# amirkdv/biseqt

Hardware: AMD Instinct MI355X
Metric: GCUPS (DP cell updates/s) banded local align (higher is better)
Workload: dtype i16

## Files before the change

biseqt_amd/_pwlib.py:

```python
import ctypes as C
import os

HERE = os.path.dirname(os.path.abspath(__file__))
PWLIB_SO = os.environ.get('PWLIB_SO', os.path.join(HERE, 'pwlib', 'pwlib.so'))
PWLIB_H = os.path.join(HERE, 'pwlib', 'pwlib.h')

STD_MODE, BANDED_MODE = 0, 1
GLOBAL, LOCAL, START_ANCHORED, END_ANCHORED, OVERLAP, START_ANCHORED_OVERLAP, \
    END_ANCHORED_OVERLAP = range(7)
B_GLOBAL, B_LOCAL, B_OVERLAP = range(3)


class intpair(C.Structure):
    _fields_ = [('i', C.c_int), ('j', C.c_int)]


class alnscores(C.Structure):
    _fields_ = [('subst_scores', C.POINTER(C.POINTER(C.c_double))),
                ('gap_open_score', C.c_double),
                ('gap_extend_score', C.c_double)]


class alnframe(C.Structure):
    _fields_ = [('origin', C.POINTER(C.c_int)),
# ... 37 lines not shown
class dptable(C.Structure):
    _fields_ = [('cells', C.POINTER(C.POINTER(dpcell))),
                ('num_rows', C.c_int),
                ('row_lens', C.POINTER(C.c_int)),
                ('prob', C.POINTER(alnprob))]


class alignment(C.Structure):
    _fields_ = [('origin_idx', C.c_int),
                ('mutant_idx', C.c_int),
                ('score', C.c_double),
                ('transcript', C.c_char_p)]


class pw_scoring(C.Structure):
    _fields_ = [('mode', C.c_int), ('type', C.c_int), ('alphabet_len', C.c_int),
                ('subst', C.POINTER(C.c_double)), ('go', C.c_double), ('ge', C.c_double)]


class pw_pair(C.Structure):
    _fields_ = [('origin_off', C.c_uint64), ('mutant_off', C.c_uint64),
                ('origin_len', C.c_int32), ('mutant_len', C.c_int32),
                ('dmin', C.c_int32), ('dmax', C.c_int32)]


class pw_result(C.Structure):
    _fields_ = [('score', C.c_double), ('opt_i', C.c_int32), ('opt_j', C.c_int32),
                ('origin_idx', C.c_int32), ('mutant_idx', C.c_int32),
                ('tx_len', C.c_int32), ('status', C.c_int32)]


PW_ST_TRACED, PW_ST_EMPTY, PW_ST_PANICK, PW_ST_BADPATH = 1, 2, 4, 8
PW_FLAG_DUMP_SCORES, PW_FLAG_FORCE_F64, PW_FLAG_FORCE_GENERIC, PW_FLAG_PROFILE = 1, 2, 4, 8
PW_FLAG_NO_PACKED16 = 16
PW_FLAG_FORCE_TILED = 32
PW_FLAG_FORCE_STRIP = 64
PW_FLAG_SHARED_ARENA = 128
PW_FLAG_NO_STRIP = 256

SIZEOF = dict(intpair=8, alnscores=24, alnframe=32, std_alnparams=4, banded_alnparams=12,
              alnprob=32, alnchoice=32, dpcell=16, dptable=32, alignment=24,
              pw_scoring=40, pw_pair=32, pw_result=32)

EXPORTS = ['dptable_init', 'dptable_solve', 'dptable_traceback', 'dptable_free',
           'pw_last_error', 'pw_device_count', 'pw_device_memory', 'pw_pool_trim', 'pw_batch_create', 'pw_batch_destroy',
           'pw_batch_init_rc', 'pw_batch_band', 'pw_batch_pair_cells', 'pw_batch_cells',
           'pw_batch_algorithmic_bytes', 'pw_batch_score_type', 'pw_batch_kernel_name', 'pw_batch_upload_arena',
           'pw_batch_arena_device', 'pw_arena_upload', 'pw_arena_free', 'pw_batch_share_arena', 'pw_host_alloc', 'pw_host_free', 'pw_batch_upload_arena_async',
           'pw_batch_results_async', 'pw_batch_transcripts_async', 'pw_batch_solve', 'pw_batch_traceback',
           'pw_batch_traceback_from', 'pw_batch_sync', 'pw_batch_results_device',
           'pw_batch_transcripts_device', 'pw_batch_transcripts_bytes', 'pw_batch_tx_slot',
           'pw_batch_results', 'pw_batch_transcripts', 'pw_batch_scores', 'pw_batch_masks', 'pw_batch_table', 'pw_batch_fill_ms',
           'pw_batch_trace_ms', 'pw_batch_pack_transcripts', 'pw_batch_packed_device', 'pw_batch_packed_offsets_device',
           'pw_batch_packed_total_async', 'pw_batch_packed', 'pw_plan_only']
SEED_EXPORTS = ['pw_seeds_create', 'pw_seeds_build', 'pw_seeds_num_rows', 'pw_seeds_is_self', 'pw_seeds_rows_device',
                'pw_seeds_rows', 'pw_seeds_count', 'pw_seeds_kmers', 'pw_seeds_band_neighbours', 'pw_seeds_graph_build', 'pw_seeds_graph_num_points', 'pw_seeds_graph_points',
                'pw_seeds_graph_counts', 'pw_seeds_graph_fetch', 'pw_seeds_graph_components', 'pw_seeds_build_ms',
                'pw_seeds_algorithmic_bytes', 'pw_seeds_destroy', 'pw_seeds_last_error']

MSEED_EXPORTS = ['pw_mseeds_create', 'pw_mseeds_build', 'pw_mseeds_num_seqs', 'pw_mseeds_num_rows', 'pw_mseeds_rows_device',
                 'pw_mseeds_rows', 'pw_mseeds_count_many', 'pw_mseeds_graph_build', 'pw_mseeds_graph_counts',
                 'pw_mseeds_graph_fetch', 'pw_mseeds_graph_components', 'pw_mseeds_build_ms', 'pw_mseeds_graph_ms',
                 'pw_mseeds_components_ms', 'pw_mseeds_count_ms', 'pw_mseeds_algorithmic_bytes', 'pw_mseeds_destroy',
                 'pw_mseeds_last_error']

OVERLAP_EXPORTS = ['pw_overlap_bands', 'pw_overlap_all_pairs', 'pw_overlap_last_ms', 'pw_overlap_last_error']


class pw_read_pair(C.Structure):
    _fields_ = [('s_off', C.c_uint64), ('t_off', C.c_uint64), ('s_len', C.c_int32), ('t_len', C.c_int32)]


def check_layout():
    for name, size in SIZEOF.items():
        assert C.sizeof(globals()[name]) == size, (name, C.sizeof(globals()[name]), size)


_lib = None


def _bind_hip_runtime():
    import sys
    choice = os.environ.get('PWLIB_HIP_RUNTIME', '')
    if choice == 'system':
        return None
    try:
        with open('/proc/self/maps') as f:
            if 'libamdhip64' in f.read():
                return None
    except OSError:
        pass
    path = choice
    if not path:
        if 'torch' in sys.modules:
            return None
        try:
            import importlib.util
            spec = importlib.util.find_spec('torch')
        except (ImportError, ValueError):
            spec = None
        if spec is None or not spec.origin:
            return None
        path = os.path.join(os.path.dirname(spec.origin), 'lib', 'libamdhip64.so')
    if not os.path.exists(path):
        return None
    try:
        return C.CDLL(path, mode=C.RTLD_GLOBAL)
# ... 31 lines not shown
    lib.pw_batch_band.argtypes = [C.c_void_p, C.c_int32, P(C.c_int32), P(C.c_int32), P(C.c_int32)]
    lib.pw_batch_pair_cells.argtypes = [C.c_void_p, C.c_int32]
    lib.pw_batch_pair_cells.restype = C.c_int64
    lib.pw_batch_cells.argtypes = [C.c_void_p]
    lib.pw_batch_cells.restype = C.c_int64
    lib.pw_batch_algorithmic_bytes.argtypes = [C.c_void_p]
    lib.pw_batch_algorithmic_bytes.restype = C.c_int64
    lib.pw_batch_score_type.argtypes = [C.c_void_p]
    lib.pw_batch_kernel_name.argtypes = [C.c_void_p]
    lib.pw_batch_kernel_name.restype = C.c_char_p
    lib.pw_batch_upload_arena.argtypes = [C.c_void_p, C.c_void_p, C.c_uint64]
    lib.pw_batch_arena_device.argtypes = [C.c_void_p]
    lib.pw_batch_arena_device.restype = C.c_void_p
    lib.pw_arena_upload.argtypes = [C.c_int, C.c_void_p, C.c_uint64]
    lib.pw_arena_upload.restype = C.c_void_p
    lib.pw_arena_free.argtypes = [C.c_int, C.c_void_p]
    lib.pw_arena_free.restype = None
    lib.pw_batch_share_arena.argtypes = [C.c_void_p, C.c_void_p]
    lib.pw_host_alloc.argtypes = [C.c_uint64]
    lib.pw_host_alloc.restype = C.c_void_p
    lib.pw_host_free.argtypes = [C.c_void_p]
    lib.pw_host_free.restype = None
    lib.pw_batch_upload_arena_async.argtypes = [C.c_void_p, C.c_void_p, C.c_uint64, C.c_void_p]
    lib.pw_batch_results_async.argtypes = [C.c_void_p, C.c_void_p, C.c_void_p]
    lib.pw_batch_transcripts_async.argtypes = [C.c_void_p, C.c_void_p, C.c_void_p]
    lib.pw_batch_solve.argtypes = [C.c_void_p, C.c_void_p]
    lib.pw_batch_traceback.argtypes = [C.c_void_p, C.c_void_p]
    lib.pw_batch_traceback_from.argtypes = [C.c_void_p, P(C.c_int32), C.c_void_p]
    lib.pw_batch_sync.argtypes = [C.c_void_p, C.c_void_p]
    lib.pw_batch_results_device.argtypes = [C.c_void_p]
    lib.pw_batch_results_device.restype = C.c_void_p
    lib.pw_batch_transcripts_device.argtypes = [C.c_void_p]
    lib.pw_batch_transcripts_device.restype = C.c_void_p
    lib.pw_batch_transcripts_bytes.argtypes = [C.c_void_p]
    lib.pw_batch_transcripts_bytes.restype = C.c_uint64
    lib.pw_batch_tx_slot.argtypes = [C.c_void_p, C.c_int32, P(C.c_uint64), P(C.c_int32)]
    lib.pw_batch_results.argtypes = [C.c_void_p, C.c_void_p]
    lib.pw_batch_transcripts.argtypes = [C.c_void_p, C.c_void_p]
    lib.pw_batch_scores.argtypes = [C.c_void_p, C.c_int32, P(C.c_double), C.c_int64]
    lib.pw_batch_table.argtypes = [C.c_void_p, C.c_int32, P(C.c_double), C.c_int64]
    lib.pw_batch_masks.argtypes = [C.c_void_p, C.c_int32, P(C.c_uint8), C.c_int64]
    lib.pw_batch_fill_ms.argtypes = [C.c_void_p]
    lib.pw_batch_fill_ms.restype = C.c_float
    lib.pw_batch_trace_ms.argtypes = [C.c_void_p]
    lib.pw_batch_trace_ms.restype = C.c_float
    lib.pw_batch_pack_transcripts.argtypes = [C.c_void_p, C.c_void_p]
    lib.pw_batch_packed_device.argtypes = [C.c_void_p]
    lib.pw_batch_packed_device.restype = C.c_void_p
    lib.pw_batch_packed_offsets_device.argtypes = [C.c_void_p]
    lib.pw_batch_packed_offsets_device.restype = C.c_void_p
    lib.pw_batch_packed_total_async.argtypes = [C.c_void_p, C.c_void_p, C.c_void_p]
    lib.pw_batch_packed.argtypes = [C.c_void_p, C.c_void_p, C.c_uint64, C.c_void_p]
    lib.pw_plan_only.argtypes = [P(pw_scoring), C.c_int32, P(pw_pair), C.c_uint64, C.c_uint32, C.c_char_p, C.c_int32, P(C.c_int32)]
    lib.pw_seeds_create.argtypes = [C.c_int, C.c_void_p, C.c_int64, C.c_void_p, C.c_int64, C.c_int, C.c_int,
                                    P(C.c_uint64), C.c_int, C.c_int]
    lib.pw_seeds_create.restype = C.c_void_p
    lib.pw_seeds_build.argtypes = [C.c_void_p, C.c_int64, C.c_void_p]
    lib.pw_seeds_num_rows.argtypes = [C.c_void_p]
    lib.pw_seeds_num_rows.restype = C.c_int64
    lib.pw_seeds_is_self.argtypes = [C.c_void_p]
    lib.pw_seeds_rows_device.argtypes = [C.c_void_p]
    lib.pw_seeds_rows_device.restype = C.c_void_p
    lib.pw_seeds_rows.argtypes = [C.c_void_p, C.c_void_p, C.c_int64]
    lib.pw_seeds_count.argtypes = [C.c_void_p, C.c_int, C.c_int32, C.c_int32, C.c_int, C.c_int32, C.c_int32]
    lib.pw_seeds_count.restype = C.c_int64
    lib.pw_seeds_kmers.argtypes = [C.c_void_p, C.c_int, C.c_void_p, C.c_int64]
    lib.pw_seeds_kmers.restype = C.c_int64
    lib.pw_seeds_band_neighbours.argtypes = [C.c_void_p, C.c_void_p, C.c_int64, C.c_void_p, C.c_int64]
    lib.pw_seeds_graph_build.argtypes = [C.c_void_p, C.c_double, C.c_double]
    lib.pw_seeds_graph_build.restype = C.c_int64
    lib.pw_seeds_graph_num_points.argtypes = [C.c_void_p]
    lib.pw_seeds_graph_num_points.restype = C.c_int64
    lib.pw_seeds_graph_points.argtypes = [C.c_void_p, C.c_void_p, C.c_int64]
    lib.pw_seeds_graph_counts.argtypes = [C.c_void_p, C.c_void_p, C.c_int64]
    lib.pw_seeds_graph_fetch.argtypes = [C.c_void_p, C.c_void_p, C.c_void_p]
    lib.pw_seeds_graph_components.argtypes = [C.c_void_p, C.c_void_p, C.c_void_p]
    lib.pw_seeds_build_ms.argtypes = [C.c_void_p]
    lib.pw_seeds_build_ms.restype = C.c_double
    lib.pw_seeds_algorithmic_bytes.argtypes = [C.c_void_p]
    lib.pw_seeds_algorithmic_bytes.restype = C.c_int64
    lib.pw_seeds_destroy.argtypes = [C.c_void_p]
    lib.pw_seeds_destroy.restype = None
    lib.pw_seeds_last_error.restype = C.c_char_p
    lib.pw_mseeds_create.argtypes = [C.c_int, C.c_void_p, C.c_void_p, C.c_int, C.c_int, C.c_int]
    lib.pw_mseeds_create.restype = C.c_void_p
    lib.pw_mseeds_build.argtypes = [C.c_void_p, C.c_int64, C.c_void_p]
    lib.pw_mseeds_num_seqs.argtypes = [C.c_void_p]
    lib.pw_mseeds_num_rows.argtypes = [C.c_void_p]
    lib.pw_mseeds_num_rows.restype = C.c_int64
    lib.pw_mseeds_rows_device.argtypes = [C.c_void_p]
    lib.pw_mseeds_rows_device.restype = C.c_void_p
    lib.pw_mseeds_rows.argtypes = [C.c_void_p, C.c_void_p, C.c_int64]
    lib.pw_mseeds_count_many.argtypes = [C.c_void_p, C.c_int64, C.c_void_p, C.c_void_p, C.c_void_p, C.c_void_p]
    lib.pw_mseeds_graph_build.argtypes = [C.c_void_p, C.c_double, C.c_double]
    lib.pw_mseeds_graph_build.restype = C.c_int64
    lib.pw_mseeds_graph_counts.argtypes = [C.c_void_p, C.c_void_p, C.c_int64]
    lib.pw_mseeds_graph_fetch.argtypes = [C.c_void_p, C.c_void_p, C.c_void_p]
    lib.pw_mseeds_graph_components.argtypes = [C.c_void_p, C.c_void_p, C.c_void_p]
    for f in ('pw_mseeds_build_ms', 'pw_mseeds_graph_ms', 'pw_mseeds_components_ms', 'pw_mseeds_count_ms'):
        getattr(lib, f).argtypes = [C.c_void_p]
        getattr(lib, f).restype = C.c_double
    lib.pw_mseeds_algorithmic_bytes.argtypes = [C.c_void_p]
    lib.pw_mseeds_algorithmic_bytes.restype = C.c_int64
    lib.pw_mseeds_destroy.argtypes = [C.c_void_p]
    lib.pw_mseeds_destroy.restype = None
    lib.pw_mseeds_last_error.restype = C.c_char_p
# ... 14 lines not shown
```

biseqt_amd/csrc/pw_launch.h:

```cpp
#ifndef PW_LAUNCH_H
#define PW_LAUNCH_H

#include <hip/hip_runtime_api.h>

#include "pw_plan.h"
#include "pw_types.h"

namespace pw {

hipError_t launch_fill(const FillParams<int32_t>& a, int variant, int bk, int nblocks, hipStream_t st);
hipError_t launch_fill(const FillParams<double>& a, int variant, int bk, int nblocks, hipStream_t st);
hipError_t launch_fill16(const FillParams<int32_t>& a, int bk, int seg, int rule, int mat, int nwaves, hipStream_t st);
hipError_t launch_fill16_mw(const FillParams<int32_t>& a, int bk, int rule, int mat, int nw, int npairs, hipStream_t st);
hipError_t launch_fill_mw(const FillParams<int32_t>& a, int variant, int bk, int nw, int nblocks, hipStream_t st);
hipError_t launch_fill_mw(const FillParams<double>& a, int variant, int bk, int nw, int nblocks, hipStream_t st);
hipError_t launch_tile(const FillParams<int32_t>& a, int variant, int pair, int ntiles, hipStream_t st);
hipError_t launch_tile(const FillParams<double>& a, int variant, int pair, int ntiles, hipStream_t st);
hipError_t launch_tile_finish(const FillParams<int32_t>& a, int pair, hipStream_t st);
hipError_t launch_tile_finish(const FillParams<double>& a, int pair, hipStream_t st);
hipError_t launch_trace(const TraceParams& p, hipStream_t st);
hipError_t launch_tx_pack(const PairDesc* pairs, const Result* results, const uint8_t* slots, int n, uint64_t* offsets,
                          uint8_t* packed, hipStream_t st);
struct StripParams;
struct StripTraceParams;
hipError_t launch_strip_fill(const StripParams& a, bool track, bool byte_rows, const uint32_t* ctl_init, int nworkers, int lds_bytes,
                             hipStream_t st);
hipError_t launch_strip_trace(const StripTraceParams& p, hipStream_t st);
hipError_t launch_xcc_census(uint32_t* d_seen8, hipStream_t st);
hipError_t launch_table_rowmajor(const void* plane, bool f64, int X, int Y, int pitch, double mul, double* out, hipStream_t st);

}
#endif
```

biseqt_amd/csrc/pw_trace.hip:

```cpp
#include "pw_device.h"

#include <stdlib.h>

namespace pw {

__global__ __launch_bounds__(64) void k_trace(const TraceParams p, const int walkers) {
  __shared__ uint32_t win[64][WIN_WORDS + 1];
  const int pair = (int)blockIdx.x * walkers + (int)threadIdx.x;
  if ((int)threadIdx.x < walkers && pair < p.npairs) trace_walk(p, pair, win[threadIdx.x]);
}

__device__ inline uint32_t bytes_equal(uint32_t w, uint32_t c4) {
  const uint32_t v = w ^ c4;
  const uint32_t t = (v & 0x7f7f7f7fu) + 0x7f7f7f7fu;
  return ~(t | v | 0x7f7f7f7fu);
}
__global__ __launch_bounds__(64) void k_trace_fixup(const TraceParams p) {
  const int pair = (int)blockIdx.x;
  const PairDesc& pd = p.pairs[pair];
  if (!pd.solvable) return;
  const Result r = p.results[pair];
  if (!(r.status & ST_TRACED) || r.tx_len <= 0) return;
  const uint8_t* oseq = p.arena + pd.o_off;
  const uint8_t* mseq = p.arena + pd.m_off;
// ... 38 lines not shown
__global__ __launch_bounds__(1024) void k_tx_offsets(const Result* __restrict__ results, int n, unsigned long long* __restrict__ offsets) {
  __shared__ unsigned long long part[1024];
  const int t = (int)threadIdx.x;
  const int per = (n + 1023) / 1024;
  const int k0 = t * per, k1 = k0 + per < n ? k0 + per : n;
  unsigned long long s = 0;
  for (int k = k0; k < k1; k++) { const int len = results[k].tx_len; s += len > 0 ? (unsigned long long)len : 0ull; }
  part[t] = s;
  __syncthreads();
  for (int off = 1; off < 1024; off <<= 1) {
    const unsigned long long v = t >= off ? part[t - off] : 0ull;
    __syncthreads();
    part[t] += v;
    __syncthreads();
  }
  unsigned long long run = t > 0 ? part[t - 1] : 0ull;
  for (int k = k0; k < k1; k++) {
    offsets[k] = run;
    const int len = results[k].tx_len;
    run += len > 0 ? (unsigned long long)len : 0ull;
  }
  if (t == 1023) offsets[n] = part[1023];
}
__global__ __launch_bounds__(64) void k_tx_pack(const PairDesc* __restrict__ pairs, const Result* __restrict__ results,
                                                const uint8_t* __restrict__ slots, const unsigned long long* __restrict__ offsets,
                                                uint8_t* __restrict__ packed) {
  const int pair = (int)blockIdx.x;
  const int len = results[pair].tx_len;
  if (len <= 0) return;
  const PairDesc& pd = pairs[pair];
  const uint8_t* src = slots + pd.tx_off + pd.tx_cap - len;
  uint8_t* dst = packed + offsets[pair];
  const int lane = (int)threadIdx.x;
  const int head = (int)((4u - (uint32_t)((uintptr_t)dst & 3u)) & 3u);
  if (lane < head && lane < len) dst[lane] = src[lane];
  const int nwords = len > head ? (len - head) >> 2 : 0;
  for (int q = lane; q < nwords; q += 64) {
    const uint8_t* sp = src + head + 4 * q;
    PackedU32 v = *(const PackedU32*)sp;
    *(uint32_t*)(dst + head + 4 * q) = v.v;
  }
  const int tail0 = head + 4 * nwords;
  if (tail0 + lane < len) dst[tail0 + lane] = src[tail0 + lane];
}
hipError_t launch_tx_pack(const PairDesc* pairs, const Result* results, const uint8_t* slots, int n, uint64_t* offsets,
                          uint8_t* packed, hipStream_t st) {
  hipLaunchKernelGGL(k_tx_offsets, dim3(1), dim3(1024), 0, st, results, n, (unsigned long long*)offsets);
  hipError_t e = hipGetLastError();
  if (e != hipSuccess || n <= 0) return e;
  hipLaunchKernelGGL(k_tx_pack, dim3((unsigned)n), dim3(64), 0, st, pairs, results, slots, (const unsigned long long*)offsets, packed);
  return hipGetLastError();
}

template <typename T>
__global__ __launch_bounds__(256) void k_table_rowmajor(const T* __restrict__ plane, int X, int Y, int pitch, double mul, double* __restrict__ out) {
  const int64_t c = (int64_t)blockIdx.x * 256 + threadIdx.x;
  if (c >= (int64_t)(X + 1) * (Y + 1)) return;
  const int x = (int)(c / (Y + 1)), y = (int)(c - (int64_t)x * (Y + 1));
  out[c] = (double)plane[(int64_t)(x - y + Y) * pitch + (x < y ? x : y)] * mul;
}
hipError_t launch_table_rowmajor(const void* plane, bool f64, int X, int Y, int pitch, double mul, double* out, hipStream_t st) {
  const int64_t n = (int64_t)(X + 1) * (Y + 1);
  const dim3 grid((unsigned)((n + 255) / 256)), blk(256);
  if (f64) hipLaunchKernelGGL((k_table_rowmajor<double>), grid, blk, 0, st, (const double*)plane, X, Y, pitch, mul, out);
  else hipLaunchKernelGGL((k_table_rowmajor<int32_t>), grid, blk, 0, st, (const int32_t*)plane, X, Y, pitch, mul, out);
  return hipGetLastError();
}

hipError_t launch_trace(const TraceParams& p, hipStream_t st) {
  if (p.npairs <= 0) return hipSuccess;
  static int walkers = 0;
  if (walkers == 0) {
    const char* e = getenv("PWLIB_WALKERS_PER_WAVE");
    walkers = e ? atoi(e) : 64;
    if (walkers < 1 || walkers > 64) walkers = 64;
  }
  hipLaunchKernelGGL(k_trace, dim3((unsigned)((p.npairs + walkers - 1) / walkers)), dim3(64), 0, st, p, walkers);
  hipError_t e = hipGetLastError();
  if (e != hipSuccess) return e;
  hipLaunchKernelGGL(k_trace_fixup, dim3((unsigned)p.npairs, (unsigned)(p.fix_segments > 0 ? p.fix_segments : 1)), dim3(64), 0, st, p);
  return hipGetLastError();
}

#define PW_DECL(TN, T) \
  hipError_t launch_fill_##TN##_bk2(const FillParams<T>&, int, int, hipStream_t);  \
  hipError_t launch_fill_##TN##_bk4(const FillParams<T>&, int, int, hipStream_t);  \
  hipError_t launch_fill_##TN##_bk8(const FillParams<T>&, int, int, hipStream_t);  \
  hipError_t launch_fill_##TN##_bk16(const FillParams<T>&, int, int, hipStream_t); \
  hipError_t launch_fill_##TN##_bk32(const FillParams<T>&, int, int, hipStream_t);
PW_DECL(i32, int32_t)
PW_DECL(f64, double)
#undef PW_DECL
#define PW_BKS(M, R, MT) M(4, R, MT) M(8, R, MT) M(12, R, MT) M(16, R, MT) M(20, R, MT) M(24, R, MT) M(28, R, MT) M(32, R, MT)
#define PW_ALL16(M) PW_BKS(M, 0, 0) PW_BKS(M, 1, 0) PW_BKS(M, 2, 0) PW_BKS(M, 3, 0) PW_BKS(M, 4, 0) PW_BKS(M, 5, 0) \
                    PW_BKS(M, 0, 1) PW_BKS(M, 1, 1) PW_BKS(M, 2, 1) PW_BKS(M, 3, 1)
#define PW_DECL16(BK, R, MT) hipError_t launch_fill16_bk##BK##_r##R##_m##MT(const FillParams<int32_t>&, int, int, hipStream_t); \
  hipError_t launch_fill16mw_bk##BK##_r##R##_m##MT(const FillParams<int32_t>&, int, int, hipStream_t);
PW_ALL16(PW_DECL16)
#undef PW_DECL16

hipError_t launch_tile_i32(const FillParams<int32_t>&, int, int, int, hipStream_t);
hipError_t launch_tile_f64(const FillParams<double>&, int, int, int, hipStream_t);
hipError_t launch_tile_finish_i32(const FillParams<int32_t>&, int, hipStream_t);
hipError_t launch_tile_finish_f64(const FillParams<double>&, int, hipStream_t);
hipError_t launch_tile(const FillParams<int32_t>& a, int variant, int pair, int ntiles, hipStream_t st) { return launch_tile_i32(a, variant, pair, ntiles, st); }
hipError_t launch_tile(const FillParams<double>& a, int variant, int pair, int ntiles, hipStream_t st) { return launch_tile_f64(a, variant, pair, ntiles, st); }
// ... 53 lines not shown
```

biseqt_amd/csrc/pwlib_api.cpp:

```cpp
#include <hip/hip_runtime.h>
#include <math.h>
#include <stdint.h>
#include <stdio.h>
#include <stdlib.h>
#include <string.h>

#include <algorithm>
#include <string>
#include <chrono>
#include <memory>
#include <mutex>
#include <thread>
#include <vector>

#include "../../include/pw_batch.h"
#include "pw_launch.h"
#include "pw_plan.h"
#include "pw_model.h"
#include "pw_hip_host.h"
#define PW_FN inline
#include "pw_strip.h"
#include <atomic>

extern "C" {
// ... 128 lines not shown
};

}

struct pw_batch {
  int device = 0;
  int32_t n = 0;
  uint32_t flags = 0;
  int mode = 0, type = 0, L = 0;
  double go = 0, ge = 0;
  std::vector<double> subst;
  bool simple = false, use_f64 = false;
  double plan_ms = 0;
  pw::PlanKnobs knobs;
  int scale_shift = 0;
  double score_mul = 1.0;
  int variant = 0, brule = 0, endrule = 0, gosign = 0;
  std::vector<pw_pair> pairs;
  std::vector<pw::Plan> plans;
  std::vector<pw::PairDesc> descs;
  std::vector<BkClass> classes;
  std::vector<pw::WaveDesc> waves;
  std::vector<int32_t> strips;
  std::vector<uint32_t> strip_ctl_init;
  PoolBuffer<uint64_t> d_fifo; size_t fifo_bytes = 0;
  DeviceBuffer d_sbest;
  DeviceBuffer d_ctl;
  std::vector<int32_t> tiled;
  DeviceBuffer d_state[2];
  int32_t st_pitch = 0;
  int packed_seg = 0, packed_rule = 0, packed_nw = 1;
  int packed_mat = 0;
  DeviceBuffer d_waves;
  int64_t cells = 0, alg_bytes = 0;
  bool on_device = false;
  PoolBuffer<uint8_t> arena; uint64_t arena_bytes = 0;
  uint8_t* d_arena = nullptr;
  bool arena_shared = false;
  PoolBuffer<pw::PairDesc> d_pairs;
  PoolBuffer<uint32_t> d_masks; uint64_t mask_words = 0;
  DeviceBuffer d_hdump; uint64_t h_elems = 0;
  PoolBuffer<pw::Result> d_results;
  PoolBuffer<uint8_t> d_tx; uint64_t tx_bytes = 0;
  DeviceBuffer d_subst;
  DeviceBuffer d_ends;
  PoolBuffer<uint8_t> d_txpacked;
  DeviceBuffer d_txoffsets;
  DeviceEvent ev_fill0, ev_fill1, ev_tr0, ev_tr1;
  bool fill_timed = false, trace_timed = false;
  std::vector<double> subst_in; double go_in = 0, ge_in = 0;
  std::vector<std::pair<int32_t, std::unique_ptr<pw_batch>>> repaired;
  std::vector<std::pair<hipStream_t, DeviceEvent>> done_events;
  bool traced = false, traced_from = false;
  std::vector<int32_t> last_ends;
  ~pw_batch();
};

pw_batch::~pw_batch() {
  repaired.clear();
  if (!on_device) return;
  (void)hipSetDevice(device);
  for (auto& se : done_events) (void)hipEventSynchronize(se.second.e);
}

namespace {

pw::PlanKnobs plan_knobs() {
  auto on = [](const char* name) { return env_int(name, 0) != 0; };
  pw::PlanKnobs k;
  k.no_dyadic = on("PWLIB_NO_DYADIC");
  k.latency_mode = env_int("PWLIB_LATENCY_MODE", -1);
  k.no_packed_mat = on("PWLIB_NO_PACKED_MAT");
  k.no_packed_anchored = on("PWLIB_NO_PACKED_ANCHORED");
  k.no_packed_overlap = on("PWLIB_NO_PACKED_OVERLAP");
  k.no_packed_mw = on("PWLIB_NO_PACKED_MW");
  k.no_strip = on("PWLIB_NO_STRIP");
  k.no_small_strip = on("PWLIB_NO_SMALL_STRIP");
  k.strip_no_byte_rows = on("PWLIB_STRIP_NO_BYTE_ROWS");
  k.no_small_tiled = on("PWLIB_NO_SMALL_TILED");
  k.mw_wide_lanes = on("PWLIB_MW_WIDE_LANES");
  k.simple_as_matrix = env_int("PWLIB_SIMPLE_AS_MATRIX", -1);
  k.no_scaled16 = on("PWLIB_NO_SCALED16");
  const char* bk = getenv("PWLIB_PACKED_BK");
  if (bk && *bk) { k.packed_bk_forced = true; k.packed_bk = atoi(bk); k.packed_bk_seg = strchr(bk, 's') != nullptr; }
  return k;
}

int batch_inputs(pw_batch* b, bool plan_only, const pw_scoring* sc, int32_t n_pairs, const pw_pair* pairs, uint64_t arena_bytes,
                 uint32_t flags) {
  if (!sc || n_pairs < 0 || (n_pairs > 0 && !pairs) || (plan_only && !sc->subst))
    return fail(plan_only ? "pw_plan_only: bad arguments" : "pw_batch_create: bad arguments");
  if (sc->mode != pw::STD_MODE && sc->mode != pw::BANDED_MODE) return fail("unknown alignment mode");
  if (sc->type < 0 || sc->type > (sc->mode == pw::STD_MODE ? 6 : 2)) return fail("unknown alignment type");
  if (sc->alphabet_len < 1 || sc->alphabet_len > 256 || !sc->subst) return fail("alphabet_len must be 1..256 with a score matrix");
  b->n = n_pairs; b->flags = flags;
  b->mode = sc->mode; b->type = sc->type; b->L = sc->alphabet_len; b->go = sc->go; b->ge = sc->ge;
  b->subst.assign(sc->subst, sc->subst + (size_t)b->L * b->L);
  b->subst_in = b->subst; b->go_in = b->go; b->ge_in = b->ge;
  b->pairs.assign(pairs, pairs + n_pairs);
  b->arena_bytes = arena_bytes;
  return 0;
}

void plan_waves(pw_batch* b, const pw::PackedLayout& p16) {
  const int ppw = p16.seg ? 64 / p16.nl : 1;
  BkClass& c = b->classes[0];
// ... 335 lines not shown
      HIP_TRY(pw::launch_tile(a, b->variant, (int)k, ntiles, st));
      cur ^= 1;
    }
    a.st_in = (const T*)b->d_state[cur].p;
    HIP_TRY(pw::launch_tile_finish(a, (int)k, st));
  }
  return 0;
}

int launch_packed_fill(pw_batch* b, hipStream_t st) {
  pw::FillParams<int32_t> a = fill_params<int32_t>(b);
  a.order = (const int32_t*)b->classes[0].d_order.p; a.waves = (const pw::WaveDesc*)b->d_waves.p;
  if (b->packed_mat) pw::packed_matrix_rows(b->subst.data(), b->L, b->packed_rule == 3, a.mat_rows, &a.mat_bias);
  if (b->packed_nw > 1) HIP_TRY(pw::launch_fill16_mw(a, b->classes[0].bk, b->packed_rule, b->packed_mat, b->packed_nw, (int)b->waves.size(), st));
  else HIP_TRY(pw::launch_fill16(a, b->classes[0].bk, b->packed_seg, b->packed_rule, b->packed_mat, (int)b->waves.size(), st));
  return 0;
}

}

extern "C" {

const char* pw_last_error(void) { return g_err.c_str(); }

void pw_pool_trim(void) { pool_drop(-1); }

int pw_device_memory(int device, uint64_t* free_bytes, uint64_t* total_bytes) {
  size_t fr = 0, tot = 0;
  HIP_TRY(hipSetDevice(device));
  HIP_TRY(hipMemGetInfo(&fr, &tot));
  if (free_bytes) *free_bytes = fr;
  if (total_bytes) *total_bytes = tot;
  return 0;
}

int pw_device_count(void) {
  int n = 0;
  if (hipGetDeviceCount(&n) != hipSuccess) return 0;
  return n;
}

pw_batch* pw_batch_create(int device, const pw_scoring* sc, int32_t n_pairs, const pw_pair* pairs,
                          uint64_t arena_bytes, uint32_t flags) {
  std::unique_ptr<pw_batch> b(new pw_batch());
  b->device = device;
  if (batch_inputs(b.get(), false, sc, n_pairs, pairs, arena_bytes, flags) != 0 || batch_plan(b.get()) != 0 ||
      batch_alloc(b.get()) != 0)
    return nullptr;
  return b.release();
}

void pw_batch_destroy(pw_batch* b) { delete b; }

int pw_plan_only(const pw_scoring* sc, int32_t n_pairs, const pw_pair* pairs, uint64_t arena_bytes, uint32_t flags,
                 char* kernel, int32_t kernel_cap, int32_t* info) {
  pw_batch b;
  b.device = -1;
  if (batch_inputs(&b, true, sc, n_pairs, pairs, arena_bytes, flags) != 0 || batch_plan(&b) != 0) return -1;
  if (kernel && kernel_cap > 0) { strncpy(kernel, pw_batch_kernel_name(&b), (size_t)kernel_cap - 1); kernel[kernel_cap - 1] = 0; }
  if (info) {
    int64_t one = 0, wg = 0;
    for (const auto& c : b.classes) (c.nw > 1 || (b.variant == pw::VAR_FAST16 && b.packed_nw > 1) ? wg : one) += (int64_t)c.order.size();
    info[0] = b.use_f64 ? 1 : 0; info[1] = b.scale_shift; info[2] = (int32_t)one; info[3] = (int32_t)wg;
    info[4] = (int32_t)b.tiled.size(); info[5] = (int32_t)b.strips.size();
    info[6] = b.variant == pw::VAR_FAST16 ? b.packed_rule : -1; info[7] = b.packed_mat;
  }
  return 0;
}

int pw_batch_init_rc(const pw_batch* b, int32_t k) { return (k < 0 || k >= b->n) ? -1 : b->plans[k].rc; }

int pw_batch_band(const pw_batch* b, int32_t k, int32_t* dmin, int32_t* dmax, int32_t* num_rows) {
  if (k < 0 || k >= b->n) return -1;
  if (dmin) *dmin = b->plans[k].dmin;
  if (dmax) *dmax = b->plans[k].dmax;
  if (num_rows) *num_rows = b->plans[k].num_rows;
  return b->plans[k].clamped;
}

int64_t pw_batch_pair_cells(const pw_batch* b, int32_t k) { return (k < 0 || k >= b->n) ? -1 : b->plans[k].cells; }
int64_t pw_batch_cells(const pw_batch* b) { return b->cells; }
int64_t pw_batch_algorithmic_bytes(const pw_batch* b) { return b->alg_bytes; }
int pw_batch_score_type(const pw_batch* b) { return b->use_f64 ? 1 : 0; }

const char* pw_batch_kernel_name(const pw_batch* b) {
  static thread_local char name[96];
  int bk = 0, nw = 1; size_t most = 0;
  for (const auto& c : b->classes) if (c.order.size() > most) { most = c.order.size(); bk = c.bk; nw = c.nw; }
  if (b->classes.empty() && b->tiled.empty() && !b->strips.empty()) {
    snprintf(name, sizeof name, "k_fill_strip<%s> x row strips", b->endrule != pw::END_CORNER ? "true" : "false");
    return name;
  }
  if (b->classes.empty() && !b->tiled.empty()) { snprintf(name, sizeof name, "k_fill_tile<%s> x time blocks", b->use_f64 ? "double" : "int"); return name; }
  const char* t = b->use_f64 ? "double" : "int";
  if (nw > 1) { snprintf(name, sizeof name, "k_fill_mw<%s, %d, ...> x %d wavefronts", t, bk, nw); return name; }
  switch (b->variant) {
    case pw::VAR_FAST16:
      if (b->packed_nw > 1) snprintf(name, sizeof name, "k_fill16_mw<%d, %d> x %d wavefronts", bk, b->packed_rule, b->packed_nw);
      else if (b->packed_rule == 3) snprintf(name, sizeof name, "k_fill16<%d, %s> x4", bk, b->packed_seg ? "true" : "false");
      else if (b->packed_rule) snprintf(name, sizeof name, "k_fill16<%d, %s, %d>", bk, b->packed_seg ? "true" : "false", b->packed_rule);
      else snprintf(name, sizeof name, "k_fill16<%d, %s>", bk, b->packed_seg ? "true" : "false");
      if (b->packed_mat) strncat(name, " matrix", sizeof name - strlen(name) - 1);
      break;
    case pw::VAR_FAST_ANY_TRACK: snprintf(name, sizeof name, "k_fill<%s, %d, true, true, false>", t, bk); break;
    case pw::VAR_FAST_TRACK: snprintf(name, sizeof name, "k_fill<%s, %d, false, true, false>", t, bk); break;
    case pw::VAR_FAST: snprintf(name, sizeof name, "k_fill<%s, %d, false, false, false>", t, bk); break;
    default: snprintf(name, sizeof name, "k_fill<%s, %d, false, true, true>", t, bk); break;
  }
  return name;
}

void* pw_arena_upload(int device, const uint8_t* host, uint64_t bytes) {
  void* p = nullptr;
  if (hipSetDevice(device) != hipSuccess || hipMalloc(&p, bytes + 16) != hipSuccess) { (void)hipGetLastError(); fail("pw_arena_upload: allocation failed"); return nullptr; }
  if (hipMemset((uint8_t*)p + bytes, 0, 16) != hipSuccess || (bytes && hipMemcpy(p, host, bytes, hipMemcpyHostToDevice) != hipSuccess)) {
    (void)hipGetLastError(); (void)hipFree(p); fail("pw_arena_upload: copy failed"); return nullptr;
  }
  return p;
}
void pw_arena_free(int device, void* p) { if (p) { (void)hipSetDevice(device); (void)hipFree(p); } }
int pw_batch_share_arena(pw_batch* b, void* dev) {
  if (!b->arena_shared) return fail("pw_batch_share_arena: the batch was not created with PW_FLAG_SHARED_ARENA");
  if (!dev) return fail("pw_batch_share_arena: null arena");
  b->d_arena = (uint8_t*)dev;
  return 0;
}

int pw_batch_upload_arena(pw_batch* b, const uint8_t* host, uint64_t bytes) {
  if (b->arena_shared) return fail("the batch shares a caller-owned arena (PW_FLAG_SHARED_ARENA): nothing to upload");
  if (bytes > b->arena_bytes) return fail("arena upload larger than the arena");
  HIP_TRY(hipSetDevice(b->device));
  if (bytes) HIP_TRY(hipMemcpy(b->d_arena, host, bytes, hipMemcpyHostToDevice));
  return 0;
}

void* pw_batch_arena_device(pw_batch* b) { return b->d_arena; }

void* pw_host_alloc(uint64_t bytes) {
  void* p = nullptr;
  if (hipHostMalloc(&p, bytes ? bytes : 1, hipHostMallocDefault) != hipSuccess) { (void)hipGetLastError(); fail("hipHostMalloc failed"); return nullptr; }
  return p;
}
void pw_host_free(void* p) { if (p) (void)hipHostFree(p); }

int pw_batch_upload_arena_async(pw_batch* b, const uint8_t* host, uint64_t bytes, void* stream) {
  if (b->arena_shared) return fail("the batch shares a caller-owned arena (PW_FLAG_SHARED_ARENA): nothing to upload");
  if (bytes > b->arena_bytes) return fail("arena upload larger than the arena");
  HIP_TRY(hipSetDevice(b->device));
  if (bytes) HIP_TRY(hipMemcpyAsync(b->d_arena, host, bytes, hipMemcpyHostToDevice, (hipStream_t)stream));
  return mark_done(b, (hipStream_t)stream);
}
int pw_batch_results_async(pw_batch* b, pw_result* out, void* stream) {
  HIP_TRY(hipSetDevice(b->device));
  if (b->n) HIP_TRY(hipMemcpyAsync(out, b->d_results.p, sizeof(pw_result) * (size_t)b->n, hipMemcpyDeviceToHost, (hipStream_t)stream));
  return mark_done(b, (hipStream_t)stream);
}
int pw_batch_transcripts_async(pw_batch* b, uint8_t* out, void* stream) {
  HIP_TRY(hipSetDevice(b->device));
  if (b->tx_bytes) HIP_TRY(hipMemcpyAsync(out, b->d_tx.p, b->tx_bytes, hipMemcpyDeviceToHost, (hipStream_t)stream));
  return mark_done(b, (hipStream_t)stream);
}

int pw_batch_solve(pw_batch* b, void* stream) {
  hipStream_t st = (hipStream_t)stream;
  if (b->arena_shared && !b->d_arena) return fail("pw_batch_solve: the batch was created with PW_FLAG_SHARED_ARENA and has no arena yet");
  HIP_TRY(hipSetDevice(b->device));
  b->traced = false; b->traced_from = false;
  if (!b->repaired.empty()) {
    HIP_TRY(hipDeviceSynchronize());
    b->repaired.clear();
  }
  if (b->flags & PW_FLAG_PROFILE) HIP_TRY(hipEventRecord(b->ev_fill0.e, st));
  int rc = b->variant == pw::VAR_FAST16 ? launch_packed_fill(b, st)
           : b->use_f64 ? launch_all_fills<double>(b, st) : launch_all_fills<int32_t>(b, st);
  if (rc == 0 && !b->strips.empty()) rc = launch_strip_fills(b, st);
  if (rc != 0) return rc;
  if (b->flags & PW_FLAG_PROFILE) { HIP_TRY(hipEventRecord(b->ev_fill1.e, st)); b->fill_timed = true; }
  return mark_done(b, st);
}

static pw_batch* repaired_sub(pw_batch* b, int32_t k) {
  for (auto& r : b->repaired) if (r.first == k) return r.second.get();
  return nullptr;
}

static int replay_trace(pw_batch* b, int32_t k, pw_batch* sub, hipStream_t st) {
  if (b->traced_from) {
    const int32_t e[2] = {b->last_ends[2 * (size_t)k], b->last_ends[2 * (size_t)k + 1]};
    if (pw_batch_traceback_from(sub, e, st) != 0) return -1;
  } else if (pw_batch_traceback(sub, st) != 0) return -1;
  const pw::PairDesc& d = b->descs[k];
  HIP_TRY(hipMemcpyAsync(b->d_results.p + k, sub->d_results.p, sizeof(pw::Result), hipMemcpyDeviceToDevice, st));
  HIP_TRY(hipMemcpyAsync(b->d_tx.p + d.tx_off, sub->d_tx.p + sub->descs[0].tx_off, (size_t)d.tx_cap, hipMemcpyDeviceToDevice, st));
  return 0;
}

static int repair_strip_pair(pw_batch* b, int32_t k) {
  pw_scoring sc;
  sc.mode = b->mode; sc.type = b->type; sc.alphabet_len = b->L; sc.subst = b->subst_in.data(); sc.go = b->go_in; sc.ge = b->ge_in;
  const uint32_t keep = b->flags & (PW_FLAG_FORCE_F64 | PW_FLAG_FORCE_GENERIC | PW_FLAG_NO_PACKED16);
  std::unique_ptr<pw_batch> owned(pw_batch_create(b->device, &sc, 1, &b->pairs[k], b->arena_bytes,
                                                  keep | PW_FLAG_SHARED_ARENA | PW_FLAG_NO_STRIP));
  pw_batch* sub = owned.get();
  if (!sub) return -1;
  if (!sub->strips.empty()) return fail("internal: the replacement of a strip pair took the strips again");
  if (pw_batch_share_arena(sub, b->d_arena) != 0 || pw_batch_solve(sub, nullptr) != 0) return -1;
  b->repaired.emplace_back(k, std::move(owned));
  if (b->traced) { if (replay_trace(b, k, sub, nullptr) != 0) return -1; }
  else HIP_TRY(hipMemcpyAsync(b->d_results.p + k, sub->d_results.p, sizeof(pw::Result), hipMemcpyDeviceToDevice, nullptr));
  HIP_TRY(hipStreamSynchronize(nullptr));
  static const bool verbose = env_int("PWLIB_TIMING", 0) != 0;
  if (verbose) fprintf(stderr, "pwlib: strip pipeline of pair %d abandoned; solved again on %s\n", (int)k, pw_batch_kernel_name(sub));
// ... 22 lines not shown
    sp.X = d.X; sp.Y = d.Y; sp.nkq = pw::strip_nkq(d.Y); sp.tx_cap = d.tx_cap; sp.gosign = b->gosign;
    HIP_TRY(pw::launch_strip_trace(sp, st));
  }
  HIP_TRY(pw::launch_trace(p, st));
  for (auto& r : b->repaired) if (replay_trace(b, r.first, r.second.get(), st) != 0) return -1;
  if (b->flags & PW_FLAG_PROFILE) { HIP_TRY(hipEventRecord(b->ev_tr1.e, st)); b->trace_timed = true; }
  return mark_done(b, st);
}

int pw_batch_traceback(pw_batch* b, void* stream) {
  HIP_TRY(hipSetDevice(b->device));
  b->traced = true; b->traced_from = false;
  return do_trace(b, nullptr, (hipStream_t)stream);
}

int pw_batch_traceback_from(pw_batch* b, const int32_t* ends_ij, void* stream) {
  HIP_TRY(hipSetDevice(b->device));
  hipStream_t st = (hipStream_t)stream;
  HIP_TRY(b->d_ends.ensure(8 * std::max<int32_t>(b->n, 1)));
  for (int32_t k = 0; k < b->n; k++) {
    if (!b->descs[k].solvable) continue;
    const int i = ends_ij[2 * k], j = ends_ij[2 * k + 1];
    if (i < 0 && j < 0) continue;
    const pw::Plan& pl = b->plans[k];
    const int X = b->pairs[k].origin_len, Y = b->pairs[k].mutant_len;
    bool ok;
    if (b->mode == pw::STD_MODE) ok = i >= 0 && i <= X && j >= 0 && j <= Y;
    else ok = i >= 0 && i < pl.num_rows && j >= 0 && j < pw::plan_len(X, Y, pl.dmin + i);
    if (!ok) return fail("traceback end cell outside the table");
  }
  HIP_TRY(hipMemcpyAsync(b->d_ends.p, ends_ij, 8 * (size_t)b->n, hipMemcpyHostToDevice, st));
  b->traced = true; b->traced_from = true;
  b->last_ends.assign(ends_ij, ends_ij + 2 * (size_t)b->n);
  return do_trace(b, (const int32_t*)b->d_ends.p, st);
}

int pw_batch_sync(pw_batch* b, void* stream) {
  HIP_TRY(hipSetDevice(b->device));
  HIP_TRY(hipStreamSynchronize((hipStream_t)stream));
  return 0;
}

void* pw_batch_results_device(pw_batch* b) { return b->d_results.p; }
void* pw_batch_transcripts_device(pw_batch* b) { return b->d_tx.p; }
uint64_t pw_batch_transcripts_bytes(const pw_batch* b) { return b->tx_bytes; }

int pw_batch_tx_slot(const pw_batch* b, int32_t k, uint64_t* off, int32_t* cap) {
  if (k < 0 || k >= b->n) return -1;
  if (off) *off = b->descs[k].tx_off;
  if (cap) *cap = b->descs[k].tx_cap;
  return 0;
}

int pw_batch_results(pw_batch* b, pw_result* out) {
  HIP_TRY(hipSetDevice(b->device));
  if (b->n) HIP_TRY(hipMemcpy(out, b->d_results.p, sizeof(pw_result) * (size_t)b->n, hipMemcpyDeviceToHost));
  for (int32_t k : b->strips)
    if ((out[k].status & PW_ST_BADPATH) && out[k].opt_i < 0 && !repaired_sub(b, k)) {
      if (env_int("PWLIB_NO_STRIP_REPAIR", 0))
        return fail("the strip pipeline of a wide pair was abandoned (a wavefront waited too long for the strip above it)");
      if (repair_strip_pair(b, k) != 0)
        return fail("the strip pipeline of a wide pair was abandoned and solving the pair again without it failed: " + std::string(g_err));
      HIP_TRY(hipMemcpy(out + k, b->d_results.p + k, sizeof(pw_result), hipMemcpyDeviceToHost));
    }
  return 0;
}

int pw_batch_transcripts(pw_batch* b, uint8_t* out) {
  HIP_TRY(hipSetDevice(b->device));
  if (b->tx_bytes) HIP_TRY(hipMemcpy(out, b->d_tx.p, b->tx_bytes, hipMemcpyDeviceToHost));
  return 0;
}

int pw_batch_pack_transcripts(pw_batch* b, void* stream) {
  HIP_TRY(hipSetDevice(b->device));
  if (!b->d_txoffsets.p) {
    HIP_TRY(b->d_txpacked.alloc(b->device, std::max<uint64_t>(b->tx_bytes, 16)));
    HIP_TRY(b->d_txoffsets.ensure(8 * ((size_t)b->n + 1)));
  }
  HIP_TRY(pw::launch_tx_pack(b->d_pairs.p, b->d_results.p, b->d_tx.p, b->n, (uint64_t*)b->d_txoffsets.p, b->d_txpacked.p,
                             (hipStream_t)stream));
  return mark_done(b, (hipStream_t)stream);
}
void* pw_batch_packed_device(pw_batch* b) { return b->d_txpacked.p; }
void* pw_batch_packed_offsets_device(pw_batch* b) { return b->d_txoffsets.p; }
int pw_batch_packed_total_async(pw_batch* b, uint64_t* host_out, void* stream) {
  if (!b->d_txoffsets.p) return fail("pw_batch_packed_total_async before pw_batch_pack_transcripts");
  HIP_TRY(hipSetDevice(b->device));
  HIP_TRY(hipMemcpyAsync(host_out, (uint64_t*)b->d_txoffsets.p + b->n, 8, hipMemcpyDeviceToHost, (hipStream_t)stream));
  return mark_done(b, (hipStream_t)stream);
}
int pw_batch_packed(pw_batch* b, uint8_t* out, uint64_t cap, uint64_t* offsets_out) {
  if (!b->d_txoffsets.p) return fail("pw_batch_packed before pw_batch_pack_transcripts");
  HIP_TRY(hipSetDevice(b->device));
  std::vector<uint64_t> off((size_t)b->n + 1);
  HIP_TRY(hipMemcpy(off.data(), b->d_txoffsets.p, 8 * off.size(), hipMemcpyDeviceToHost));
  if (offsets_out) memcpy(offsets_out, off.data(), 8 * off.size());
  if (out) {
    if (off[b->n] > cap) return fail("packed transcripts: buffer too small");
    if (off[b->n]) HIP_TRY(hipMemcpy(out, b->d_txpacked.p, off[b->n], hipMemcpyDeviceToHost));
  }
  return 0;
}

int pw_batch_scores(pw_batch* b, int32_t k, double* out, int64_t n) {
  if (!(b->flags & PW_FLAG_DUMP_SCORES) || k < 0 || k >= b->n || !b->descs[k].solvable) return fail("no score plane");
  const pw::PairDesc& d = b->descs[k];
  const int64_t want = (int64_t)d.ndiag * d.h_pitch;
  if (n < want) return fail("score buffer too small");
  HIP_TRY(hipSetDevice(b->device));
  if (b->use_f64) {
    HIP_TRY(hipMemcpy(out, (double*)b->d_hdump.p + d.h_off, 8 * (size_t)want, hipMemcpyDeviceToHost));
    for (int64_t i = 0; i < want; i++) out[i] *= b->score_mul;
  } else {
    std::vector<int32_t> tmp((size_t)want);
    HIP_TRY(hipMemcpy(tmp.data(), (int32_t*)b->d_hdump.p + d.h_off, 4 * (size_t)want, hipMemcpyDeviceToHost));
    for (int64_t i = 0; i < want; i++) out[i] = (double)tmp[(size_t)i] * b->score_mul;
  }
  return 0;
}

int pw_batch_masks(pw_batch* b, int32_t k, uint8_t* out, int64_t n) {
  if (k < 0 || k >= b->n || !b->descs[k].solvable) return fail("no mask plane for this pair");
// ... 307 lines not shown
```

include/pw_batch.h:

```cpp
#ifndef PW_BATCH_H
#define PW_BATCH_H

#include <stdint.h>

#ifdef __cplusplus
extern "C" {
#endif

typedef struct pw_batch pw_batch;

typedef struct {
  int mode;
  int type;
  int alphabet_len;
  const double* subst;
  double go, ge;
} pw_scoring;

typedef struct {
  uint64_t origin_off;
  uint64_t mutant_off;
  int32_t origin_len;
  int32_t mutant_len;
  int32_t dmin, dmax;
} pw_pair;

typedef struct {
  double score;
  int32_t opt_i, opt_j;
  int32_t origin_idx;
  int32_t mutant_idx;
  int32_t tx_len;
  int32_t status;
} pw_result;

#define PW_ST_TRACED 1
#define PW_ST_EMPTY 2
#define PW_ST_PANICK 4
#define PW_ST_BADPATH 8

#define PW_FLAG_DUMP_SCORES 1
#define PW_FLAG_FORCE_F64 2
#define PW_FLAG_FORCE_GENERIC 4
#define PW_FLAG_PROFILE 8
#define PW_FLAG_NO_PACKED16 16
#define PW_FLAG_FORCE_TILED 32
#define PW_FLAG_FORCE_STRIP 64
#define PW_FLAG_SHARED_ARENA 128
#define PW_FLAG_NO_STRIP 256

const char* pw_last_error(void);
int pw_device_count(void);
int pw_device_memory(int device, uint64_t* free_bytes, uint64_t* total_bytes);

void pw_pool_trim(void);

pw_batch* pw_batch_create(int device, const pw_scoring* scoring, int32_t n_pairs, const pw_pair* pairs,
                          uint64_t arena_bytes, uint32_t flags);
void pw_batch_destroy(pw_batch* b);

int pw_plan_only(const pw_scoring* scoring, int32_t n_pairs, const pw_pair* pairs, uint64_t arena_bytes, uint32_t flags,
                 char* kernel, int32_t kernel_cap, int32_t* info);

int pw_batch_init_rc(const pw_batch* b, int32_t k);
int pw_batch_band(const pw_batch* b, int32_t k, int32_t* dmin, int32_t* dmax, int32_t* num_rows);
int64_t pw_batch_pair_cells(const pw_batch* b, int32_t k);
int64_t pw_batch_cells(const pw_batch* b);
int64_t pw_batch_algorithmic_bytes(const pw_batch* b);
int pw_batch_score_type(const pw_batch* b);
const char* pw_batch_kernel_name(const pw_batch* b);

int pw_batch_upload_arena(pw_batch* b, const uint8_t* host_arena, uint64_t bytes);
void* pw_batch_arena_device(pw_batch* b);
void* pw_arena_upload(int device, const uint8_t* host_arena, uint64_t bytes);
void pw_arena_free(int device, void* dev_arena);
int pw_batch_share_arena(pw_batch* b, void* dev_arena);
void* pw_host_alloc(uint64_t bytes);
void pw_host_free(void* p);
int pw_batch_upload_arena_async(pw_batch* b, const uint8_t* host_arena, uint64_t bytes, void* stream);
int pw_batch_results_async(pw_batch* b, pw_result* host_out, void* stream);
int pw_batch_transcripts_async(pw_batch* b, uint8_t* host_out, void* stream);

int pw_batch_solve(pw_batch* b, void* stream);
int pw_batch_traceback(pw_batch* b, void* stream);
int pw_batch_traceback_from(pw_batch* b, const int32_t* ends_ij, void* stream);
int pw_batch_sync(pw_batch* b, void* stream);

void* pw_batch_results_device(pw_batch* b);
void* pw_batch_transcripts_device(pw_batch* b);
uint64_t pw_batch_transcripts_bytes(const pw_batch* b);
int pw_batch_tx_slot(const pw_batch* b, int32_t k, uint64_t* off, int32_t* cap);
int pw_batch_results(pw_batch* b, pw_result* host_out);
int pw_batch_transcripts(pw_batch* b, uint8_t* host_out);
int pw_batch_pack_transcripts(pw_batch* b, void* stream);
void* pw_batch_packed_device(pw_batch* b);
void* pw_batch_packed_offsets_device(pw_batch* b);
int pw_batch_packed_total_async(pw_batch* b, uint64_t* host_out, void* stream);
int pw_batch_packed(pw_batch* b, uint8_t* host_out, uint64_t cap, uint64_t* offsets_out);
int pw_batch_scores(pw_batch* b, int32_t k, double* host_out, int64_t n);
int pw_batch_masks(pw_batch* b, int32_t k, uint8_t* host_out, int64_t n);
int pw_batch_table(pw_batch* b, int32_t k, double* host_out, int64_t n);

float pw_batch_fill_ms(pw_batch* b);
float pw_batch_trace_ms(pw_batch* b);

#ifdef __cplusplus
}
#endif
#endif
```

Before: 2641.

## Copy only used transcript bytes to pinned host memory with a zero-copy kernel

Instead of a hipMemcpy of the whole transcript slot buffer, a per-pair kernel writes only the used tail of each slot directly into mapped pinned host memory, using 16-byte or 4-byte vector stores with alignment head and tail handling. Device pointers for host buffers are cached per batch and invalidated through an epoch counter bumped on pw_host_free. The aim is to cut PCIe traffic when slots are much larger than the actual transcripts. The cost is a lookup on each call and fine-grained writes over the bus, and slot bytes outside the used span are no longer copied.

Result: no change. 2632 (-0.3%).

```diff
diff --git a/biseqt_amd/_pwlib.py b/biseqt_amd/_pwlib.py
--- a/biseqt_amd/_pwlib.py
+++ b/biseqt_amd/_pwlib.py
@@ -113,7 +113,7 @@
            'pw_batch_transcripts_device', 'pw_batch_transcripts_bytes', 'pw_batch_tx_slot',
            'pw_batch_results', 'pw_batch_transcripts', 'pw_batch_scores', 'pw_batch_masks', 'pw_batch_table', 'pw_batch_fill_ms',
            'pw_batch_trace_ms', 'pw_batch_pack_transcripts', 'pw_batch_packed_device', 'pw_batch_packed_offsets_device',
-           'pw_batch_packed_total_async', 'pw_batch_packed', 'pw_plan_only']
+           'pw_batch_packed_total_async', 'pw_batch_packed', 'pw_plan_only', 'pw_batch_plan', 'pw_batch_tx_span']
 SEED_EXPORTS = ['pw_seeds_create', 'pw_seeds_build', 'pw_seeds_num_rows', 'pw_seeds_is_self', 'pw_seeds_rows_device',
                 'pw_seeds_rows', 'pw_seeds_count', 'pw_seeds_kmers', 'pw_seeds_band_neighbours', 'pw_seeds_graph_build', 'pw_seeds_graph_num_points', 'pw_seeds_graph_points',
                 'pw_seeds_graph_counts', 'pw_seeds_graph_fetch', 'pw_seeds_graph_components', 'pw_seeds_build_ms',
@@ -251,6 +251,9 @@
     lib.pw_batch_packed_total_async.argtypes = [C.c_void_p, C.c_void_p, C.c_void_p]
     lib.pw_batch_packed.argtypes = [C.c_void_p, C.c_void_p, C.c_uint64, C.c_void_p]
     lib.pw_plan_only.argtypes = [P(pw_scoring), C.c_int32, P(pw_pair), C.c_uint64, C.c_uint32, C.c_char_p, C.c_int32, P(C.c_int32)]
+    lib.pw_batch_plan.argtypes = [P(pw_scoring), C.c_int32, P(pw_pair), C.c_uint64, C.c_uint32]
+    lib.pw_batch_plan.restype = C.c_void_p
+    lib.pw_batch_tx_span.argtypes = [C.c_void_p, C.c_int32, C.c_int32, C.c_uint64, C.c_int32, P(C.c_uint64), P(C.c_int32)]
     lib.pw_seeds_create.argtypes = [C.c_int, C.c_void_p, C.c_int64, C.c_void_p, C.c_int64, C.c_int, C.c_int,
                                     P(C.c_uint64), C.c_int, C.c_int]
     lib.pw_seeds_create.restype = C.c_void_p
diff --git a/biseqt_amd/csrc/pw_launch.h b/biseqt_amd/csrc/pw_launch.h
--- a/biseqt_amd/csrc/pw_launch.h
+++ b/biseqt_amd/csrc/pw_launch.h
@@ -21,6 +21,22 @@
 hipError_t launch_trace(const TraceParams& p, hipStream_t st);
 hipError_t launch_tx_pack(const PairDesc* pairs, const Result* results, const uint8_t* slots, int n, uint64_t* offsets,
                           uint8_t* packed, hipStream_t st);
+struct TxSpan {
+  uint64_t begin;
+  int32_t len, head, nvec, tail;
+};
+constexpr inline TxSpan tx_span(uint64_t tx_off, int32_t tx_cap, int32_t tx_len, uint64_t dst_base, int32_t vec) {
+  TxSpan s{0, 0, 0, 0, 0};
+  if (tx_len <= 0 || tx_cap <= 0) return s;
+  s.len = tx_len < tx_cap ? tx_len : tx_cap;
+  s.begin = tx_off + (uint64_t)(tx_cap - s.len);
+  const int32_t to_boundary = (int32_t)(((uint64_t)vec - ((dst_base + s.begin) & (uint64_t)(vec - 1))) & (uint64_t)(vec - 1));
+  s.head = to_boundary < s.len ? to_boundary : s.len;
+  s.nvec = (s.len - s.head) / vec;
+  s.tail = s.len - s.head - s.nvec * vec;
+  return s;
+}
+hipError_t launch_tx_to_host(const PairDesc* pairs, const Result* results, const uint8_t* slots, int n, uint8_t* dst, hipStream_t st);
 struct StripParams;
 struct StripTraceParams;
 hipError_t launch_strip_fill(const StripParams& a, bool track, bool byte_rows, const uint32_t* ctl_init, int nworkers, int lds_bytes,
diff --git a/biseqt_amd/csrc/pw_trace.hip b/biseqt_amd/csrc/pw_trace.hip
--- a/biseqt_amd/csrc/pw_trace.hip
+++ b/biseqt_amd/csrc/pw_trace.hip
@@ -114,6 +114,38 @@
   return hipGetLastError();
 }
 
+template <bool WIDE>
+__global__ __launch_bounds__(64) void k_tx_to_host(const PairDesc* __restrict__ pairs, const Result* __restrict__ results,
+                                                   const uint8_t* __restrict__ slots, uint8_t* __restrict__ host) {
+  const int pair = (int)blockIdx.x;
+  const int tx_len = results[pair].tx_len;
+  if (tx_len <= 0) return;
+  const PairDesc& pd = pairs[pair];
+  const TxSpan s = tx_span(pd.tx_off, pd.tx_cap, tx_len, (uint64_t)(uintptr_t)host, WIDE ? 16 : 4);
+  const uint8_t* src = slots + s.begin;
+  uint8_t* dst = host + s.begin;
+  const int lane = (int)threadIdx.x;
+  if (lane < s.head) dst[lane] = src[lane];
+  for (int q = lane; q < s.nvec; q += 64) {
+    if (WIDE) {
+      *(uint4*)(dst + s.head + 16 * q) = *(const uint4*)(src + s.head + 16 * q);
+    } else {
+      PackedU32 v = *(const PackedU32*)(src + s.head + 4 * q);
+      *(uint32_t*)(dst + s.head + 4 * q) = v.v;
+    }
+  }
+  const int tail0 = s.len - s.tail;
+  if (lane < s.tail) dst[tail0 + lane] = src[tail0 + lane];
+}
+hipError_t launch_tx_to_host(const PairDesc* pairs, const Result* results, const uint8_t* slots, int n, uint8_t* dst, hipStream_t st) {
+  if (n <= 0) return hipSuccess;
+  if ((((uintptr_t)slots ^ (uintptr_t)dst) & 15u) == 0)
+    hipLaunchKernelGGL((k_tx_to_host<true>), dim3((unsigned)n), dim3(64), 0, st, pairs, results, slots, dst);
+  else
+    hipLaunchKernelGGL((k_tx_to_host<false>), dim3((unsigned)n), dim3(64), 0, st, pairs, results, slots, dst);
+  return hipGetLastError();
+}
+
 template <typename T>
 __global__ __launch_bounds__(256) void k_table_rowmajor(const T* __restrict__ plane, int X, int Y, int pitch, double mul, double* __restrict__ out) {
   const int64_t c = (int64_t)blockIdx.x * 256 + threadIdx.x;
diff --git a/biseqt_amd/csrc/pwlib_api.cpp b/biseqt_amd/csrc/pwlib_api.cpp
--- a/biseqt_amd/csrc/pwlib_api.cpp
+++ b/biseqt_amd/csrc/pwlib_api.cpp
@@ -204,6 +204,9 @@
   std::vector<std::pair<int32_t, std::unique_ptr<pw_batch>>> repaired;
   std::vector<std::pair<hipStream_t, DeviceEvent>> done_events;
   bool traced = false, traced_from = false;
+  struct TxTarget { const uint8_t* host; uint8_t* dev; uint64_t epoch; };
+  std::vector<TxTarget> tx_targets;
+  int tx_path_told = 0;
   std::vector<int32_t> last_ends;
   ~pw_batch();
 };
@@ -645,6 +648,13 @@
 
 void pw_batch_destroy(pw_batch* b) { delete b; }
 
+pw_batch* pw_batch_plan(const pw_scoring* sc, int32_t n_pairs, const pw_pair* pairs, uint64_t arena_bytes, uint32_t flags) {
+  std::unique_ptr<pw_batch> b(new pw_batch());
+  b->device = -1;
+  if (batch_inputs(b.get(), true, sc, n_pairs, pairs, arena_bytes, flags) != 0 || batch_plan(b.get()) != 0) return nullptr;
+  return b.release();
+}
+
 int pw_plan_only(const pw_scoring* sc, int32_t n_pairs, const pw_pair* pairs, uint64_t arena_bytes, uint32_t flags,
                  char* kernel, int32_t kernel_cap, int32_t* info) {
   pw_batch b;
@@ -729,12 +739,14 @@
 
 void* pw_batch_arena_device(pw_batch* b) { return b->d_arena; }
 
+static std::atomic<uint64_t> g_host_epoch{1};
+
 void* pw_host_alloc(uint64_t bytes) {
   void* p = nullptr;
   if (hipHostMalloc(&p, bytes ? bytes : 1, hipHostMallocDefault) != hipSuccess) { (void)hipGetLastError(); fail("hipHostMalloc failed"); return nullptr; }
   return p;
 }
-void pw_host_free(void* p) { if (p) (void)hipHostFree(p); }
+void pw_host_free(void* p) { if (p) { g_host_epoch.fetch_add(1); (void)hipHostFree(p); } }
 
 int pw_batch_upload_arena_async(pw_batch* b, const uint8_t* host, uint64_t bytes, void* stream) {
   if (b->arena_shared) return fail("the batch shares a caller-owned arena (PW_FLAG_SHARED_ARENA): nothing to upload");
@@ -748,9 +760,49 @@
   if (b->n) HIP_TRY(hipMemcpyAsync(out, b->d_results.p, sizeof(pw_result) * (size_t)b->n, hipMemcpyDeviceToHost, (hipStream_t)stream));
   return mark_done(b, (hipStream_t)stream);
 }
+static uint8_t* tx_host_target(pw_batch* b, uint8_t* out) {
+  if (env_int("PWLIB_TX_HOST_KERNEL", 1) == 0) return nullptr;
+  const uint64_t epoch = g_host_epoch.load();
+  for (auto& t : b->tx_targets)
+    if (t.host == out) {
+      if (t.epoch == epoch) return t.dev;
+      t = b->tx_targets.back(); b->tx_targets.pop_back();
+      break;
+    }
+  hipPointerAttribute_t at;
+  memset(&at, 0, sizeof at);
+  uint8_t* dev = nullptr;
+  if (hipPointerGetAttributes(&at, out) == hipSuccess) {
+    void* d = nullptr;
+    if (at.type == hipMemoryTypeHost && !at.isManaged) {
+      if (hipHostGetDevicePointer(&d, out, 0) == hipSuccess) dev = (uint8_t*)d;
+      else (void)hipGetLastError();
+    }
+  } else {
+    (void)hipGetLastError();
+  }
+  if (b->tx_targets.size() >= 64) b->tx_targets.erase(b->tx_targets.begin());
+  b->tx_targets.push_back({out, dev, epoch});
+  return dev;
+}
+
+static int download_transcripts(pw_batch* b, uint8_t* out, hipStream_t st) {
+  if (!b->tx_bytes) return 0;
+  uint8_t* dev = tx_host_target(b, out);
+  if (dev) HIP_TRY(pw::launch_tx_to_host(b->d_pairs.p, b->d_results.p, b->d_tx.p, b->n, dev, st));
+  else HIP_TRY(hipMemcpyAsync(out, b->d_tx.p, b->tx_bytes, hipMemcpyDeviceToHost, st));
+  const int path = dev ? 1 : 2;
+  if (b->tx_path_told != path && env_int("PWLIB_TIMING", 0) != 0) {
+    b->tx_path_told = path;
+    if (dev) fprintf(stderr, "pwlib timing: batch of %d pairs: transcripts to the host by k_tx_to_host (the ops alone, of %llu slot bytes)\n", b->n, (unsigned long long)b->tx_bytes);
+    else fprintf(stderr, "pwlib timing: batch of %d pairs: transcripts to the host by hipMemcpy (all %llu slot bytes)\n", b->n, (unsigned long long)b->tx_bytes);
+  }
+  return 0;
+}
+
 int pw_batch_transcripts_async(pw_batch* b, uint8_t* out, void* stream) {
   HIP_TRY(hipSetDevice(b->device));
-  if (b->tx_bytes) HIP_TRY(hipMemcpyAsync(out, b->d_tx.p, b->tx_bytes, hipMemcpyDeviceToHost, (hipStream_t)stream));
+  if (download_transcripts(b, out, (hipStream_t)stream) != 0) return -1;
   return mark_done(b, (hipStream_t)stream);
 }
 
@@ -879,6 +931,14 @@
   return 0;
 }
 
+int pw_batch_tx_span(const pw_batch* b, int32_t k, int32_t tx_len, uint64_t dst_base, int32_t vec, uint64_t* begin, int32_t* head_nvec_tail) {
+  if (k < 0 || k >= b->n || (vec != 4 && vec != 16)) return -1;
+  const pw::TxSpan s = pw::tx_span(b->descs[k].tx_off, b->descs[k].tx_cap, tx_len, dst_base, vec);
+  if (begin) *begin = s.begin;
+  if (head_nvec_tail) { head_nvec_tail[0] = s.head; head_nvec_tail[1] = s.nvec; head_nvec_tail[2] = s.tail; }
+  return s.len;
+}
+
 int pw_batch_results(pw_batch* b, pw_result* out) {
   HIP_TRY(hipSetDevice(b->device));
   if (b->n) HIP_TRY(hipMemcpy(out, b->d_results.p, sizeof(pw_result) * (size_t)b->n, hipMemcpyDeviceToHost));
@@ -895,7 +955,8 @@
 
 int pw_batch_transcripts(pw_batch* b, uint8_t* out) {
   HIP_TRY(hipSetDevice(b->device));
-  if (b->tx_bytes) HIP_TRY(hipMemcpy(out, b->d_tx.p, b->tx_bytes, hipMemcpyDeviceToHost));
+  if (download_transcripts(b, out, nullptr) != 0) return -1;
+  HIP_TRY(hipStreamSynchronize(nullptr));
   return 0;
 }
 
diff --git a/include/pw_batch.h b/include/pw_batch.h
--- a/include/pw_batch.h
+++ b/include/pw_batch.h
@@ -61,6 +61,7 @@
 
 int pw_plan_only(const pw_scoring* scoring, int32_t n_pairs, const pw_pair* pairs, uint64_t arena_bytes, uint32_t flags,
                  char* kernel, int32_t kernel_cap, int32_t* info);
+pw_batch* pw_batch_plan(const pw_scoring* scoring, int32_t n_pairs, const pw_pair* pairs, uint64_t arena_bytes, uint32_t flags);
 
 int pw_batch_init_rc(const pw_batch* b, int32_t k);
 int pw_batch_band(const pw_batch* b, int32_t k, int32_t* dmin, int32_t* dmax, int32_t* num_rows);
@@ -92,6 +93,7 @@
 int pw_batch_tx_slot(const pw_batch* b, int32_t k, uint64_t* off, int32_t* cap);
 int pw_batch_results(pw_batch* b, pw_result* host_out);
 int pw_batch_transcripts(pw_batch* b, uint8_t* host_out);
+int pw_batch_tx_span(const pw_batch* b, int32_t k, int32_t tx_len, uint64_t dst_base, int32_t vec, uint64_t* begin, int32_t* head_nvec_tail);
 int pw_batch_pack_transcripts(pw_batch* b, void* stream);
 void* pw_batch_packed_device(pw_batch* b);
 void* pw_batch_packed_offsets_device(pw_batch* b);
```
